# anilkeshwani/speech-integration

Hardware: AMD Instinct MI355X
Metric: train_tokens_per_sec (higher is better)
Workload: dtype bf16; 1 GPU; Llama-3.2-1B +5000 DSUs (V=133258), SFT step fwd+bwd+AdamW, seq_len=2048, batch=8/GPU, grad_accum=1, 16 layers, random-init weights, MLS-shaped synthetic DSU sequences; global_batch=8, seq_len=2048, parallelism=dp1

## Files before the change

### include/ssi_hip.h

```cpp
#ifndef SSI_HIP_H
#define SSI_HIP_H

#include <stdint.h>

#ifdef __cplusplus
extern "C" {
#endif

#define SSI_ABI_VERSION 9

enum { SSI_F32 = 0, SSI_BF16 = 1 };
enum { SSI_OK = 0, SSI_ERR_ARG = 1, SSI_ERR_UNSUPPORTED = 2, SSI_ERR_WORKSPACE = 3, SSI_ERR_HIP = 1000  };
enum { SSI_GEMM_NT = 0, SSI_GEMM_NN = 1, SSI_GEMM_TN = 2 };
enum { SSI_TILES_STATIC = 0, SSI_TILES_DYNAMIC = 1 };
int ssi_set_gemm_tile_order(int mode);

enum { SSI_IMPL_AUTO = 0, SSI_IMPL_GENERIC = 1, SSI_IMPL_MFMA = 2,
       SSI_IMPL_MFMA_WG8 = 3  };

int ssi_abi_version(void);
const char* ssi_last_error(void);
int ssi_set_impl(int impl);

int ssi_embed_fwd(const int64_t* tokens, const void* table, void* out, int64_t n_tok, int64_t dim, int64_t vocab,
                  int dtype, void* stream);
int64_t ssi_embed_bwd_workspace_bytes(int64_t vocab);
int ssi_embed_bwd(const int64_t* tokens, const void* dout, void* dtable, int64_t n_tok, int64_t dim, int64_t vocab,
                  int dtype, void* workspace, int64_t workspace_bytes, void* stream);

int ssi_rmsnorm_fwd(const void* x, const void* scale, void* y, float* rstd, int64_t rows, int64_t dim, float eps,
                    int dtype, void* stream);
int64_t ssi_rmsnorm_bwd_workspace_bytes(int64_t rows, int64_t dim);
int ssi_rmsnorm_bwd(const void* dy, const void* x, const void* scale, const float* rstd, const void* dres, void* dx,
                    void* dscale, int accumulate_dscale, int64_t rows, int64_t dim, int dtype, void* workspace,
                    int64_t workspace_bytes, void* stream);

int ssi_rope_inplace(void* x, int64_t ld, int64_t rows, int64_t seq_len, int n_heads_rot, int head_dim,
                     const float* table, int64_t table_len, const int32_t* positions, int inverse, int dtype,
                     void* stream);

int ssi_gemm_rope(int64_t M, int64_t N, int64_t K, const void* A, int64_t lda, const void* B, int64_t ldb, void* C, int64_t ldc,
                  int64_t seq_len, int n_heads_rot, int head_dim, const float* rope_table, int64_t table_len,
                  const int32_t* positions, int dtype, void* stream);

int ssi_attn_fwd(const void* qkv, int64_t ld, void* out, float* lse, int64_t batch, int64_t seq, int n_heads,
                 int n_kv, int head_dim, int dtype, void* stream);
int ssi_attn_bwd(const void* qkv, int64_t ld, const void* out, const void* dout, const float* lse, void* dqkv,
                 float* delta, int64_t batch, int64_t seq, int n_heads, int n_kv, int head_dim, int dtype,
                 void* stream);

int ssi_attn_varlen_fwd(const void* qkv, int64_t ld, void* out, float* lse, const int32_t* doc_start, const int32_t* doc_end,
                        int64_t batch, int64_t seq, int n_heads, int n_kv, int head_dim, int dtype, void* stream);
int ssi_attn_varlen_bwd(const void* qkv, int64_t ld, const void* out, const void* dout, const float* lse, void* dqkv,
                        float* delta, const int32_t* doc_start, const int32_t* doc_end, int64_t batch, int64_t seq,
                        int n_heads, int n_kv, int head_dim, int dtype, void* stream);

int ssi_doc_ranges(const int64_t* input_pos, int64_t batch, int64_t seq, int64_t max_pos, int32_t* positions, int32_t* doc_start,
                   int32_t* doc_end, int32_t* n_clamped, void* stream);

int ssi_attn_varlen_bwd_rope(const void* qkv, int64_t ld, const void* out, const void* dout, const float* lse, void* dqkv,
                             float* delta, const int32_t* doc_start, const int32_t* doc_end, const float* rope_table,
                             int64_t table_len, const int32_t* positions, int64_t batch, int64_t seq, int n_heads, int n_kv,
                             int head_dim, int dtype, void* stream);

int64_t ssi_attn_bwd_workspace_bytes(int64_t batch, int64_t seq, int n_heads, int n_kv, int head_dim, int dtype);
int ssi_attn_varlen_bwd_ws(const void* qkv, int64_t ld, const void* out, const void* dout, const float* lse, void* dqkv,
                           float* delta, const int32_t* doc_start, const int32_t* doc_end, const float* rope_table,
                           int64_t table_len, const int32_t* positions, int64_t batch, int64_t seq, int n_heads, int n_kv,
                           int head_dim, int dtype, void* workspace, int64_t workspace_bytes, void* stream);

enum { SSI_ATTN_KERNEL_DQ = 0, SSI_ATTN_KERNEL_DKV = 1 };
enum { SSI_ATTN_MODE_AUTO = 0, SSI_ATTN_MODE_OLD = 1, SSI_ATTN_MODE_NEW = 2, SSI_ATTN_MODE_NO_HEAD_SPLIT = 3 };
int ssi_set_attn_impl(int which, int mode);
enum { SSI_ATTN_USED_DQ2 = 1, SSI_ATTN_USED_DKV2 = 2, SSI_ATTN_USED_HEAD_SPLIT = 4, SSI_ATTN_USED_PLAN = 8 };
int ssi_attn_last_dispatch(void);

enum { SSI_ATTN_PLAN_HEADER = 16, SSI_ATTN_PLAN_FORCE = 1, SSI_ATTN_PLAN_SPLIT_ALL = 2  };
int64_t ssi_attn_plan_words(int64_t batch, int64_t seq, int64_t n_docs);
int64_t ssi_attn_plan_workspace_bytes(const int32_t* host_plan_header);
int64_t ssi_attn_plan_build(const int32_t* host_doc_row, const int32_t* host_doc_start, const int32_t* host_doc_end, int64_t n_docs,
                            int64_t batch, int64_t seq, int n_heads, int n_kv, int flags, int32_t* host_plan, int64_t plan_words);
// ... 59 lines not shown
```

### speech-integration_amd/csrc/embed_ce.hip

```cpp
#include "common_hip.h"

template <typename T>
__global__ __launch_bounds__(256) void embed_fwd_kernel(const int64_t* __restrict__ tokens, const T* __restrict__ table,
                                                        T* __restrict__ out, int64_t n_tok, int dim, int64_t vocab) {
    constexpr int N = Vec16<T>::N;
    const int nvec = dim / N;
    for (int64_t t = blockIdx.x; t < n_tok; t += gridDim.x) {
        const int64_t tok = tokens[t];
        const bool ok = tok >= 0 && tok < vocab;
        for (int v = threadIdx.x; v < nvec; v += 256) {
            Vec16<T> a;
            if (ok) a = load16(table + tok * dim + v * N);
            else
#pragma unroll
                for (int i = 0; i < N; ++i) a.set(i, 0.f);
            store16(out + t * dim + v * N, a);
        }
    }
}

extern "C" int ssi_embed_fwd(const int64_t* tokens, const void* table, void* out, int64_t n_tok, int64_t dim,
                             int64_t vocab, int dtype, void* stream) {
    if (n_tok == 0) return SSI_OK;
    SSI_CHECK_ARG(tokens && table && out && n_tok > 0 && dim > 0 && dim % 8 == 0 && vocab > 0);
// ... 85 lines not shown
                for (int k = 0; k < MAXV; ++k) {
                    const bool ok = row_ok && lane + k * 64 < nvec;
#pragma unroll
                    for (int i = 0; i < N; ++i) acc[k][i] += ok ? a[u][k].get(i) : 0.f;
                }
            }
        }
        found += n;
    }
    T* dst = dtable + tok * dim;
#pragma unroll
    for (int k = 0; k < MAXV; ++k) {
        const int v = lane + k * 64;
        if (v < nvec) {
            Vec16<T> a = load16(dst + v * N);
#pragma unroll
            for (int i = 0; i < N; ++i) a.set(i, a.get(i) + acc[k][i]);
            store16(dst + v * N, a);
        }
    }
}

static inline int64_t embed_ws_vocab_slots(int64_t vocab) { return ssi_align_up(vocab, 64); }
extern "C" int64_t ssi_embed_bwd_workspace_bytes(int64_t vocab) { return 2 * embed_ws_vocab_slots(vocab) * (int64_t)sizeof(int); }

template <typename T>
static int launch_embed_bwd(const int64_t* tokens, const T* dout, T* dtable, int64_t n_tok, int dim, int64_t vocab,
                            const int* first, const int* count, hipStream_t st) {
    const int64_t vec_per_lane = ssi_cdiv(dim / Vec16<T>::N, 64);
    const dim3 grid((unsigned)ssi_cdiv(n_tok, 4));
    if (vec_per_lane <= 1) hipLaunchKernelGGL((embed_bwd_kernel<T, 1>), grid, dim3(256), 0, st, tokens, dout, dtable, n_tok, dim, vocab, first, count);
    else if (vec_per_lane <= 2) hipLaunchKernelGGL((embed_bwd_kernel<T, 2>), grid, dim3(256), 0, st, tokens, dout, dtable, n_tok, dim, vocab, first, count);
    else if (vec_per_lane <= 4) hipLaunchKernelGGL((embed_bwd_kernel<T, 4>), grid, dim3(256), 0, st, tokens, dout, dtable, n_tok, dim, vocab, first, count);
    else if (vec_per_lane <= 8) hipLaunchKernelGGL((embed_bwd_kernel<T, 8>), grid, dim3(256), 0, st, tokens, dout, dtable, n_tok, dim, vocab, first, count);
    else { ssi_set_error("embed_bwd: dim %d too large", dim); return SSI_ERR_UNSUPPORTED; }
    return SSI_OK;
}

extern "C" int ssi_embed_bwd(const int64_t* tokens, const void* dout, void* dtable, int64_t n_tok, int64_t dim,
                             int64_t vocab, int dtype, void* workspace, int64_t workspace_bytes, void* stream) {
    if (n_tok == 0) return SSI_OK;
    SSI_CHECK_ARG(tokens && dout && dtable && n_tok > 0 && n_tok < (1LL << 31) && dim > 0 && dim % 8 == 0 && vocab > 0);
    if (!workspace || workspace_bytes < ssi_embed_bwd_workspace_bytes(vocab)) { ssi_set_error("embed_bwd: workspace too small"); return SSI_ERR_WORKSPACE; }
    auto st = (hipStream_t)stream;
    int* first = (int*)workspace;
    int* count = first + embed_ws_vocab_slots(vocab);
    hipError_t e = hipMemsetAsync(first, 0x7f, embed_ws_vocab_slots(vocab) * sizeof(int), st);
    if (e == hipSuccess) e = hipMemsetAsync(count, 0, embed_ws_vocab_slots(vocab) * sizeof(int), st);
    if (e != hipSuccess) { ssi_set_error("embed_bwd: memset failed: %s", hipGetErrorString(e)); return SSI_ERR_HIP + (int)e; }
    hipLaunchKernelGGL(embed_index_kernel, dim3((unsigned)ssi_cdiv(n_tok, 256)), dim3(256), 0, st, tokens, n_tok, vocab, first, count);
    SSI_LAUNCH_CHECK();
    int rc = SSI_OK;
    SSI_DISPATCH_DTYPE(dtype, rc = launch_embed_bwd<T>(tokens, (const T*)dout, (T*)dtable, n_tok, (int)dim, vocab, first, count, st));
    if (rc) return rc;
    SSI_LAUNCH_CHECK();
    return SSI_OK;
}

template <typename T>
__global__ __launch_bounds__(512) void ce_fwd_kernel(T* __restrict__ logits, int64_t ld, const int64_t* __restrict__ labels,
                                                     int64_t vocab, int64_t ignore_index, float* __restrict__ row_loss,
                                                     float* __restrict__ row_lse, int write_grad, const float* __restrict__ row_weight) {
    constexpr int N = Vec16<T>::N;
    __shared__ float red[16];
    const int64_t row = blockIdx.x;
    T* lr = logits + row * ld;
    const int64_t label = labels[row];
    const bool valid = label != ignore_index && label >= 0 && label < vocab;
    const int64_t nvec = ld / N;
    if (!valid) {
        if (threadIdx.x == 0) { row_loss[row] = 0.f; if (row_lse) row_lse[row] = 0.f; }
        if (write_grad) {
            Vec16<T> z;
#pragma unroll
            for (int i = 0; i < N; ++i) z.set(i, 0.f);
            for (int64_t v = threadIdx.x; v < nvec; v += 512) store16(lr + v * N, z);
        }
        return;
    }
    float m = -INFINITY, s = 0.f;
    for (int64_t v = threadIdx.x; v < nvec; v += 512) {
        Vec16<T> a = load16(lr + v * N);
        float lm = -INFINITY;
#pragma unroll
        for (int i = 0; i < N; ++i) if (v * N + i < vocab) lm = fmaxf(lm, a.get(i));
        if (lm > m) { s *= expf(m - lm); m = lm; }
#pragma unroll
        for (int i = 0; i < N; ++i) if (v * N + i < vocab) s += expf(a.get(i) - m);
    }
    const float gm = block_max(m, red);
    s = (m == -INFINITY) ? 0.f : s * expf(m - gm);
    const float gs = block_sum(s, red);
    const float lse = gm + logf(gs);
    const float w = row_weight ? row_weight[row] : 1.f;
    if (threadIdx.x == 0) {
        row_loss[row] = w * (lse - to_f32<T>(lr[label]));
        if (row_lse) row_lse[row] = lse;
    }
    if (!write_grad) return;
    __syncthreads();
    for (int64_t v = threadIdx.x; v < nvec; v += 512) {
        Vec16<T> a = load16(lr + v * N), o;
#pragma unroll
        for (int i = 0; i < N; ++i) {
            const int64_t c = v * N + i;
            float g = 0.f;
// ... 179 lines not shown
```

### speech-integration_amd/ssi/_lib.py

```python

from __future__ import annotations

import ctypes
import os
from ctypes import POINTER, c_char_p, c_double, c_float, c_int, c_int32, c_int64, c_void_p

import torch

_HERE = os.path.dirname(os.path.abspath(__file__))
LIB_PATH = os.environ.get("SSI_HIP_LIB") or os.path.join(os.path.dirname(_HERE), "libssi_hip.so")

SSI_F32, SSI_BF16 = 0, 1
GEMM_NT, GEMM_NN, GEMM_TN = 0, 1, 2
IMPL_AUTO, IMPL_GENERIC, IMPL_MFMA, IMPL_MFMA_WG8 = 0, 1, 2, 3
TILES_STATIC, TILES_DYNAMIC = 0, 1
ABI_VERSION = 9
ATTN_KERNEL_DQ, ATTN_KERNEL_DKV = 0, 1
ATTN_MODE_AUTO, ATTN_MODE_OLD, ATTN_MODE_NEW, ATTN_MODE_NO_HEAD_SPLIT = 0, 1, 2, 3
ATTN_USED_DQ2, ATTN_USED_DKV2, ATTN_USED_HEAD_SPLIT, ATTN_USED_PLAN = 1, 2, 4, 8
ATTN_PLAN_HEADER, ATTN_PLAN_FORCE, ATTN_PLAN_SPLIT_ALL = 16, 1, 2

_P = c_void_p
PROTOTYPES = {
    "ssi_abi_version": (c_int, []),
    "ssi_last_error": (c_char_p, []),
    "ssi_set_impl": (c_int, [c_int]),
    "ssi_set_attn_impl": (c_int, [c_int, c_int]),
    "ssi_attn_last_dispatch": (c_int, []),
    "ssi_embed_fwd": (c_int, [_P, _P, _P, c_int64, c_int64, c_int64, c_int, _P]),
    "ssi_embed_bwd_workspace_bytes": (c_int64, [c_int64]),
    "ssi_embed_bwd": (c_int, [_P, _P, _P, c_int64, c_int64, c_int64, c_int, _P, c_int64, _P]),
    "ssi_rmsnorm_fwd": (c_int, [_P, _P, _P, _P, c_int64, c_int64, c_float, c_int, _P]),
    "ssi_rmsnorm_bwd_workspace_bytes": (c_int64, [c_int64, c_int64]),
    "ssi_rmsnorm_bwd": (c_int, [_P, _P, _P, _P, _P, _P, _P, c_int, c_int64, c_int64, c_int, _P, c_int64, _P]),
    "ssi_rope_inplace": (c_int, [_P, c_int64, c_int64, c_int64, c_int, c_int, _P, c_int64, _P, c_int, c_int, _P]),
    "ssi_gemm_rope": (c_int, [c_int64, c_int64, c_int64, _P, c_int64, _P, c_int64, _P, c_int64, c_int64, c_int, c_int, _P, c_int64, _P,
                              c_int, _P]),
    "ssi_attn_fwd": (c_int, [_P, c_int64, _P, _P, c_int64, c_int64, c_int, c_int, c_int, c_int, _P]),
    "ssi_attn_bwd": (c_int, [_P, c_int64, _P, _P, _P, _P, _P, c_int64, c_int64, c_int, c_int, c_int, c_int, _P]),
    "ssi_set_gemm_tile_order": (c_int, [c_int]),
    "ssi_attn_varlen_fwd": (c_int, [_P, c_int64, _P, _P, _P, _P, c_int64, c_int64, c_int, c_int, c_int, c_int, _P]),
    "ssi_attn_varlen_bwd": (c_int, [_P, c_int64, _P, _P, _P, _P, _P, _P, _P, c_int64, c_int64, c_int, c_int, c_int, c_int, _P]),
    "ssi_attn_varlen_bwd_rope": (c_int, [_P, c_int64, _P, _P, _P, _P, _P, _P, _P, _P, c_int64, _P, c_int64, c_int64, c_int, c_int, c_int,
                                         c_int, _P]),
    "ssi_attn_bwd_workspace_bytes": (c_int64, [c_int64, c_int64, c_int, c_int, c_int, c_int]),
    "ssi_attn_varlen_bwd_ws": (c_int, [_P, c_int64, _P, _P, _P, _P, _P, _P, _P, _P, c_int64, _P, c_int64, c_int64, c_int, c_int, c_int,
                                       c_int, _P, c_int64, _P]),
    "ssi_attn_plan_words": (c_int64, [c_int64, c_int64, c_int64]),
    "ssi_attn_plan_workspace_bytes": (c_int64, [_P]),
    "ssi_attn_plan_build": (c_int64, [_P, _P, _P, c_int64, c_int64, c_int64, c_int, c_int, c_int, _P, c_int64]),
    "ssi_attn_varlen_bwd_plan": (c_int, [_P, c_int64, _P, _P, _P, _P, _P, _P, _P, _P, c_int64, _P, c_int64, c_int64, c_int, c_int, c_int,
                                         c_int, _P, c_int64, _P, _P, _P]),
    "ssi_doc_ranges": (c_int, [_P, c_int64, c_int64, c_int64, _P, _P, _P, _P, _P]),
    "ssi_swiglu_fwd": (c_int, [_P, _P, c_int64, c_int64, c_int, _P]),
    "ssi_swiglu_bwd": (c_int, [_P, _P, _P, c_int64, c_int64, c_int, _P]),
    "ssi_gemm": (c_int, [c_int, c_int64, c_int64, c_int64, _P, c_int64, _P, c_int64, _P, c_int64, _P, c_float, _P,
                         c_int, c_int, _P]),
    "ssi_gemm_splitk_workspace_bytes": (c_int64, [c_int64, c_int64, c_int]),
    "ssi_gemm_splitk": (c_int, [c_int, c_int64, c_int64, c_int64, _P, c_int64, _P, c_int64, _P, c_int64, _P, c_float, _P,
                                c_int, c_int, c_int, _P, c_int64, _P]),
    "ssi_gemm_batched": (c_int, [c_int, c_int, c_int64, c_int64, c_int64, _P, c_int64, c_int64, _P, c_int64, c_int64, _P, c_int64, c_int64,
                                 c_float, _P, c_int, c_int, _P]),
    "ssi_gemm_swiglu_fwd": (c_int, [c_int64, c_int64, c_int64, _P, c_int64, _P, c_int64, _P, c_int64, _P, c_int64, c_int, _P]),
    "ssi_gemm_swiglu_bwd": (c_int, [c_int, c_int64, c_int64, c_int64, _P, c_int64, _P, c_int64, _P, c_int64, _P, c_int64, _P, c_int,
                                    _P]),
    "ssi_transpose": (c_int, [_P, c_int64, _P, c_int64, c_int64, c_int64, c_int, _P]),
    "ssi_ce_fwd": (c_int, [_P, c_int64, _P, c_int64, c_int64, c_int64, _P, _P, c_int, c_int, _P]),
    "ssi_ce_fwd_weighted": (c_int, [_P, c_int64, _P, _P, c_int64, c_int64, c_int64, _P, _P, c_int, c_int, _P]),
    "ssi_ce_reduce": (c_int, [_P, _P, c_int64, c_int64, c_int64, _P, _P]),
    "ssi_lmhead_ce_fwd": (c_int, [_P, c_int64, _P, c_int64, _P, c_int64, c_int64, c_int64, c_int64, c_int64, _P, c_int64, _P, _P, c_int, c_int, _P]),
    "ssi_lmhead_ce_bwd": (c_int, [_P, c_int64, _P, c_int64, _P, c_int64, _P, c_int64, c_int64, c_int64, _P, c_int64, _P, c_int64, c_int, c_int, _P]),
    "ssi_count_tokens": (c_int, [_P, _P, c_int64, _P, c_int, c_int64, c_int64, _P, _P]),
    "ssi_scale_inplace": (c_int, [_P, c_int64, c_float, _P, c_int, _P]),
    "ssi_sumsq_workspace_bytes": (c_int64, [c_int64]),
    "ssi_sumsq": (c_int, [_P, c_int64, c_int, _P, _P, c_int64, _P]),
    "ssi_adamw_step": (c_int, [_P, _P, _P, _P, c_int64, c_double, c_double, c_double, c_double, c_double, c_int64, _P, c_int,
                               c_int, _P]),
}

_lib = None


class HipLibraryError(RuntimeError):
    pass
# ... 55 lines not shown
```

### speech-integration_amd/ssi/model.py

```python

from __future__ import annotations

import os

import logging
import math
from typing import Any, Optional

import torch
from torch import Tensor, nn

from . import _lib, ops
from .constants import CROSS_ENTROPY_IGNORE_IDX, PRECISION_STR_TO_DTYPE
from .llama_configs import ConfigLlama3_2
from .ops import GEMM_NN, GEMM_NT, GEMM_TN

LOGGER = logging.getLogger(__name__)

VOCAB_ALIGN = 256


def _align(n: int, a: int) -> int:
    return (n + a - 1) // a * a

# ... 273 lines not shown
        M, N = c.shape
        K = a.shape[1]
        mfma = self.split_small_grids and self.dtype == torch.bfloat16 and self._mfma_shapes() and M % 256 == 0 and N % 256 == 0
        if mfma and self.split_tail_only and layout in (GEMM_NT, GEMM_NN):
            tm, tn = M // 256, N // 256
            rounds = (tm * tn) // 256
            m_main = (rounds * 256) // tn
            if rounds >= 1 and 0 < m_main < tm and (tm - m_main) * tn <= 192:
                rows = m_main * 256
                ops.gemm(layout, a[:rows], b, c[:rows], residual=None if residual is None else residual[:rows])
                self._gemm(layout, a[rows:], b, c[rows:], None if residual is None else residual[rows:])
                return
        splits = ops.splitk_choice(M, N, K) if mfma else 1
        if splits > 1:
            wsk = self._arena.get("ws.splitk.nt", (splits * M * N,), torch.float32)
            ops.gemm_splitk(layout, a, b, c, splits, wsk, residual=residual)
        else:
            ops.gemm(layout, a, b, c, residual=residual)

    def build_attn_plan(self, input_pos: Tensor, force: bool = False):
        from . import attn_plan
        if input_pos is None or input_pos.is_cuda or input_pos.dim() != 2 or not self._mfma_shapes() or self.head_dim != 64:
            return None
        B, S = input_pos.shape
        if self.num_heads != 4 * self.num_kv_heads or self.padded_seq_len(B, S) != S or S % 128:
            return None
        return attn_plan.plan_from_input_pos(input_pos, self.num_heads, self.num_kv_heads, force=force)

    def _forward_hidden(self, tokens: Tensor, save: bool, input_pos: Optional[Tensor] = None, attn_plan=None) -> Tensor:
        B, S = tokens.shape
        pos = ds = de = None
        self.position_errors = None
        plan = None
        if input_pos is not None and save:
            if attn_plan is None and not input_pos.is_cuda:
                attn_plan = self.build_attn_plan(input_pos)
            if attn_plan is not None and attn_plan.matches(B, S, self.num_heads, self.num_kv_heads) and self._mfma_shapes():
                plan = attn_plan.to_device(tokens.device)
        if input_pos is not None:
            if input_pos.shape != tokens.shape:
                raise ValueError("input_pos must have the shape of tokens")
            if not input_pos.is_cuda and int(input_pos.max()) >= self._rope.shape[0]:
                raise ValueError("input_pos exceeds the RoPE cache")
            self.position_errors = torch.zeros(1, dtype=torch.int32, device=tokens.device)
            pos, ds, de = ops.doc_ranges(input_pos.to(tokens.device), self._rope.shape[0] - 1, self.position_errors)
        T, D, I = B * S, self.embed_dim, self.intermediate_dim
        H, KV, hd, dt, A = self.num_heads, self.num_kv_heads, self.head_dim, self.dtype, self._arena
        if pos is None and S > self._rope.shape[0]:
            raise ValueError(f"sequence length {S} exceeds the RoPE cache ({self._rope.shape[0]})")
        tok = tokens.reshape(-1).contiguous()
        L = self.num_layers
        h = A.get("h0" if save else "h0.x", (T, D), dt)
        ops.embed_fwd(tok, self._view("emb"), h, self.vocab_size)
        for l in range(L):
            sfx = f"{l}" if save else "x"
            xn1 = A.get("xn1.all", (L, T, D), dt)[l] if save else A.get("xn1.x", (T, D), dt)
            rstd1 = A.get(f"rstd1.{sfx}", (T,), torch.float32)
            ops.rmsnorm_fwd(h, self._view(f"L{l}.sa_norm"), xn1, rstd1, self.norm_eps)
            qkv = A.get(f"qkv.{sfx}", (T, self.qkv_dim), dt)
            ops.gemm_rope(xn1, self._view(f"L{l}.wqkv"), qkv, S, H + KV, hd, self._rope, positions=pos)
            att = A.get("att.all", (L, T, H * hd), dt)[l] if save else A.get("att.x", (T, H * hd), dt)
            lse = A.get(f"lse.{sfx}", (B * H * S,), torch.float32)
            ops.attn_fwd(qkv, att, lse, B, S, H, KV, hd, ds, de)
            hmid = A.get(f"hmid.{sfx}", (T, D), dt)
            self._gemm(GEMM_NT, att, self._view(f"L{l}.wo"), hmid, residual=h)
            xn2 = A.get(f"xn2.{sfx}", (T, D), dt)
            rstd2 = A.get(f"rstd2.{sfx}", (T,), torch.float32)
            ops.rmsnorm_fwd(hmid, self._view(f"L{l}.mlp_norm"), xn2, rstd2, self.norm_eps)
            gu = A.get(f"gu.{sfx}", (T, 2 * I), dt)
            act = A.get(f"act.{sfx}", (T, I), dt)
            ops.gemm_swiglu_fwd(xn2, self._view(f"L{l}.w13"), gu, act)
            hn_name = f"h{l + 1}" if save else f"hx{l & 1}"
            hnext = A.get(hn_name, (T, D), dt)
            self._gemm(GEMM_NT, act, self._view(f"L{l}.w2"), hnext, residual=hmid)
            h = hnext
        hn = A.get("hn" if save else "hn.x", (T, D), dt)
        rstdf = A.get("rstdf" if save else "rstdf.x", (T,), torch.float32)
        ops.rmsnorm_fwd(h, self.norm.scale, hn, rstdf, self.norm_eps)
        if save:
            self._fwd_generation += 1
            self._saved = {"tok": tok, "B": B, "S": S, "gen": self._fwd_generation, "pos": pos, "ds": ds, "de": de, "plan": plan}
        return hn

    def _backward_hidden(self, d_hn: Tensor, gen: int) -> None:
        sv = self._saved
        if sv is None or sv["gen"] != gen:
            raise RuntimeError("HipLlamaDecoder: backward called for a forward whose activations were overwritten; "
                               "run backward before the next training forward")
        B, S, tok = sv["B"], sv["S"], sv["tok"]
        pos, ds, de, plan = sv["pos"], sv["ds"], sv["de"], sv.get("plan")
        T, D, I = B * S, self.embed_dim, self.intermediate_dim
        H, KV, hd, dt, A = self.num_heads, self.num_kv_heads, self.head_dim, self.dtype, self._arena
        L = self.num_layers
        G = self._flat_grad
        self._finish_pending_exchange()
        acc = self._window_accumulates()
        gv = lambda name: self._view(name, None, G)
        ws = A.get("ws.rms", (max(ops.rmsnorm_bwd_workspace_bytes(T, D), 16),), torch.uint8)

        def wgrad(dy: Tensor, x: Tensor, name: str) -> None:
            g = gv(name)
            splits = ops.splitk_choice(g.shape[0], g.shape[1], T) if (dt == torch.bfloat16 and T % 64 == 0) else 1
            if splits > 1:
                wsk = A.get("ws.splitk", (splits * g.shape[0] * g.shape[1],), torch.float32)
                ops.gemm_splitk(GEMM_TN, dy, x, g, splits, wsk, accumulate=acc)
            else:
                ops.gemm(GEMM_TN, dy, x, g, accumulate=acc)

        sync = self.grad_sync if (self.grad_sync is not None and self.sync_this_backward) else None
        listener, self.bucket_listener = (self.bucket_listener if self.sync_this_backward else None), None

        def announce(name: str) -> None:
            if sync:
                sync.bucket_ready(*self._bucket_by_name[name])
            if listener is not None:
                listener(*self._bucket_by_name[name])

        Gp = self.wgrad_group
        if sync and Gp != self._bucket_group:
            raise RuntimeError("wgrad_group was changed after construction: the data-parallel buckets were laid out for the old grouping")
        defer = (Gp > 1 and dt == torch.bfloat16 and self._mfma_shapes() and T % 128 == 0 and T >= 256
                 and ops.splitk_choice(D, H * hd, T) > 1 and ops.splitk_choice(self.qkv_dim, D, T) > 1)
        xn1_all, att_all = A.get("xn1.all", (L, T, D), dt), A.get("att.all", (L, T, H * hd), dt)
        if defer:
            dhmid_all, dqkv_all = A.get("dh.b.all", (Gp, T, D), dt), A.get("dqkv.all", (Gp, T, self.qkv_dim), dt)
            lstride = (self._slices["L1.wqkv"][0] - self._slices["L0.wqkv"][0]) if L > 1 else 0

        def flush_attention_wgrads(l_lo: int) -> None:
            n = min(Gp, L - l_lo)
            g_o = torch.as_strided(G, (n, D, H * hd), (lstride, H * hd, 1), self._slices[f"L{l_lo}.wo"][0])
            g_qkv = torch.as_strided(G, (n, self.qkv_dim, D), (lstride, D, 1), self._slices[f"L{l_lo}.wqkv"][0])
            ops.gemm_batched(GEMM_TN, dhmid_all[:n], att_all[l_lo:l_lo + n], g_o, accumulate=acc)
            ops.gemm_batched(GEMM_TN, dqkv_all[:n], xn1_all[l_lo:l_lo + n], g_qkv, accumulate=acc)

        def dgrad(dy: Tensor, name: str, dx: Tensor) -> None:
            self._gemm(GEMM_NN, dy, self._view(name), dx)

        ws_bytes = ops.attn_bwd_workspace_bytes(B, S, H, KV, hd, dt) if T > 0 else 0
        if plan is not None:
            ws_bytes = max(ws_bytes, plan.workspace_bytes)
        attn_ws = A.get("ws.attn", (ws_bytes,), torch.uint8) if ws_bytes else None
        dh = A.get("dh.a", (T, D), dt)
        ops.rmsnorm_bwd(d_hn, A.get(f"h{L}", (T, D), dt), self.norm.scale, A.get("rstdf", (T,), torch.float32), None, dh,
                        gv("norm"), ws, accumulate=acc)
        announce("norm")
        for l in reversed(range(L)):
            xn1, xn2 = xn1_all[l], A.get(f"xn2.{l}", (T, D), dt)
            qkv, att = A.get(f"qkv.{l}", (T, self.qkv_dim), dt), att_all[l]
            hmid, gu, act = A.get(f"hmid.{l}", (T, D), dt), A.get(f"gu.{l}", (T, 2 * I), dt), A.get(f"act.{l}", (T, I), dt)
            h_in = A.get(f"h{l}", (T, D), dt)
            wgrad(dh, act, f"L{l}.w2")
            dgu = A.get("dgu", (T, 2 * I), dt)
            ops.gemm_swiglu_bwd(GEMM_NN, dh, self._view(f"L{l}.w2"), gu, dgu, A.get("dact", (T, I), dt))
            dxn = A.get("dxn", (T, D), dt)
            dgrad(dgu, f"L{l}.w13", dxn)
            wgrad(dgu, xn2, f"L{l}.w13")
            dhmid = dhmid_all[l % Gp] if defer else A.get("dh.b", (T, D), dt)
            ops.rmsnorm_bwd(dxn, hmid, self._view(f"L{l}.mlp_norm"), A.get(f"rstd2.{l}", (T,), torch.float32), dh, dhmid,
                            gv(f"L{l}.mlp_norm"), ws, accumulate=acc)
            datt = A.get("datt", (T, H * hd), dt)
            dgrad(dhmid, f"L{l}.wo", datt)
            if not defer:
                wgrad(dhmid, att, f"L{l}.wo")
            dqkv = dqkv_all[l % Gp] if defer else A.get("dqkv", (T, self.qkv_dim), dt)
            delta = A.get("delta", (B * H * S,), torch.float32)
            ops.attn_bwd(qkv, att, datt, A.get(f"lse.{l}", (B * H * S,), torch.float32), dqkv, delta, B, S, H, KV, hd, ds, de,
                         rope_table=self._rope, positions=pos, workspace=attn_ws, plan=plan)
            dgrad(dqkv, f"L{l}.wqkv", dxn)
            if not defer:
                wgrad(dqkv, xn1, f"L{l}.wqkv")
            ops.rmsnorm_bwd(dxn, h_in, self._view(f"L{l}.sa_norm"), A.get(f"rstd1.{l}", (T,), torch.float32), dhmid, dh,
                            gv(f"L{l}.sa_norm"), ws, accumulate=acc)
            announce(f"L{l}.mlp")
            if defer and l % Gp == 0:
                flush_attention_wgrads(l)
            if l % self._bucket_group == 0:
                announce(f"attn.{l}")
        ws_e = A.get("ws.emb", (max(_lib.load().ssi_embed_bwd_workspace_bytes(self.vocab_size), 16),), torch.uint8)
        if not acc and not self._emb_grad_written:
            gv("emb").zero_()
        ops.embed_bwd(tok, dh, gv("emb"), self.vocab_size, ws_e)
        self._grads_dirty, self._grads_stale, self._emb_grad_written = True, False, False
        announce("emb")
        self._saved = None
        self.attach_grads()

    def _head_logits(self, hn: Tensor, arena_name: Optional[str] = None) -> Tensor:
        T = hn.shape[0]
        if arena_name is None:
            logits = torch.empty((T, self.vocab_pad), dtype=self.dtype, device=self.device)
        else:
            logits = self._arena.get(arena_name, (T, self.vocab_pad), self.dtype)
        ops.gemm(GEMM_NT, hn, self._view("emb"), logits)
        return logits

    def _head_backward(self, dlogits: Tensor, hn: Tensor, alpha_dev: Optional[Tensor]) -> Tensor:
        T, D = hn.shape
        self._finish_pending_exchange()
        acc = self._window_accumulates()
        d_hn = self._arena.get("d_hn", (T, D), self.dtype)
        ops.gemm(GEMM_NN, dlogits, self._view("emb"), d_hn, alpha_dev=alpha_dev)
        g_emb = self._view("emb", None, self._flat_grad)
        rows_main = self._head_wgrad_main_rows(T)
        if rows_main:
            Vp = self.vocab_pad
            ops.gemm(GEMM_TN, dlogits[:, :rows_main], hn, g_emb[:rows_main], alpha_dev=alpha_dev, accumulate=acc)
            tail, splits = Vp - rows_main, self._head_wgrad_tail_splits
            wsk = self._arena.get("ws.splitk.head", (splits * tail * D,), torch.float32)
            ops.gemm_splitk(GEMM_TN, dlogits[:, rows_main:], hn, g_emb[rows_main:], splits, wsk, alpha_dev=alpha_dev, accumulate=acc)
        else:
            ops.gemm(GEMM_TN, dlogits, hn, g_emb, alpha_dev=alpha_dev, accumulate=acc)
        self._emb_grad_written = True
        return d_hn

    _head_wgrad_tail_splits = 3

    def _head_wgrad_main_rows(self, T: int, n_cu: int = 256) -> int:
        if os.environ.get("SSI_HEAD_WGRAD_TAIL", "1") == "0" or self.dtype != torch.bfloat16 or not self._mfma_shapes() or T % 128 or T < 64 * 6 * self._head_wgrad_tail_splits:
            return 0
        tm, tn = self.vocab_pad // 256, self.embed_dim // 256
        full_rounds = (tm * tn) // n_cu
        if full_rounds == 0 or (full_rounds * n_cu) % tn:
            return 0
        tail_tiles = tm * tn - full_rounds * n_cu
        if tail_tiles == 0 or 2 * tail_tiles >= n_cu or tail_tiles * self._head_wgrad_tail_splits > n_cu:
            return 0
        return full_rounds * n_cu // tn * 256

    def _check_inputs(self, tokens: Tensor, mask, encoder_input, encoder_mask, input_pos) -> Tensor:
        if encoder_input is not None or encoder_mask is not None:
            raise NotImplementedError("no encoder inputs: the reference's model is decoder-only (ssi/model.py:34)")
        if mask is not None and input_pos is None:
            raise NotImplementedError("a dense attention mask is never materialised: packed batches pass input_pos, from which "
                                      "the block-causal mask follows (ssi/data/packed.py)")
# ... 174 lines not shown
```

### speech-integration_amd/ssi/ops.py

```python

from __future__ import annotations

import torch
from typing import Optional
from torch import Tensor

from . import _lib
from ._lib import GEMM_NN, GEMM_NT, GEMM_TN, check, dtype_code, ptr, stream_ptr

__all__ = ["lmhead_ce_fwd", "lmhead_ce_bwd", "doc_ranges", "embed_fwd", "embed_bwd", "rmsnorm_fwd", "rmsnorm_bwd", "rope_", "attn_fwd", "attn_bwd", "attn_bwd_workspace_bytes", "swiglu_fwd",
           "swiglu_bwd", "gemm", "gemm_splitk", "splitk_choice", "gemm_swiglu_fwd", "gemm_swiglu_bwd", "transpose", "ce_fwd", "ce_reduce", "count_tokens", "scale_", "sumsq", "adamw_step", "set_impl", "set_attn_impl", "attn_last_dispatch",
           "GEMM_NT", "GEMM_NN", "GEMM_TN"]


def set_impl(impl: int) -> int:
    return _lib.load().ssi_set_impl(impl)


def set_attn_impl(which: int, mode: int) -> int:
    return _lib.load().ssi_set_attn_impl(which, mode)


def attn_last_dispatch() -> int:
    return _lib.load().ssi_attn_last_dispatch()


def _byte_ws(nbytes: int, like: Tensor) -> Tensor:
    return torch.empty(max(int(nbytes), 16), dtype=torch.uint8, device=like.device)


def embed_fwd(tokens: Tensor, table: Tensor, out: Tensor, vocab: int) -> None:
    n, dim = tokens.numel(), table.shape[1]
    assert tokens.dtype == torch.int64 and tokens.is_contiguous() and out.is_contiguous() and table.stride(1) == 1
    assert table.stride(0) == dim and out.shape[-1] == dim and out.numel() == n * dim and out.dtype == table.dtype
    check(_lib.load().ssi_embed_fwd(ptr(tokens), ptr(table), ptr(out), n, dim, vocab, dtype_code(table.dtype),
                                    stream_ptr()), "ssi_embed_fwd")


def embed_bwd(tokens: Tensor, dout: Tensor, dtable: Tensor, vocab: int, workspace: Tensor | None = None) -> None:
    lib = _lib.load()
    n, dim = tokens.numel(), dtable.shape[1]
    assert tokens.dtype == torch.int64 and tokens.is_contiguous() and dout.is_contiguous() and dtable.stride(0) == dim
    need = lib.ssi_embed_bwd_workspace_bytes(vocab)
    if workspace is None or workspace.numel() * workspace.element_size() < need:
        workspace = _byte_ws(need, dout)
    check(lib.ssi_embed_bwd(ptr(tokens), ptr(dout), ptr(dtable), n, dim, vocab, dtype_code(dtable.dtype), ptr(workspace),
                            workspace.numel() * workspace.element_size(), stream_ptr()), "ssi_embed_bwd")


def rmsnorm_fwd(x: Tensor, scale: Tensor, y: Tensor, rstd: Tensor | None, eps: float) -> None:
    dim = x.shape[-1]
    rows = x.numel() // dim
    assert x.is_contiguous() and y.is_contiguous() and scale.is_contiguous() and scale.numel() == dim
    assert rstd is None or (rstd.dtype == torch.float32 and rstd.numel() >= rows)
    check(_lib.load().ssi_rmsnorm_fwd(ptr(x), ptr(scale), ptr(y), ptr(rstd), rows, dim, eps, dtype_code(x.dtype),
                                      stream_ptr()), "ssi_rmsnorm_fwd")


def rmsnorm_bwd_workspace_bytes(rows: int, dim: int) -> int:
    return _lib.load().ssi_rmsnorm_bwd_workspace_bytes(rows, dim)


def rmsnorm_bwd(dy: Tensor, x: Tensor, scale: Tensor, rstd: Tensor, dres: Tensor | None, dx: Tensor, dscale: Tensor,
                workspace: Tensor | None = None, accumulate: bool = True) -> None:
    lib = _lib.load()
    dim = x.shape[-1]
    rows = x.numel() // dim
    assert dy.is_contiguous() and x.is_contiguous() and dx.is_contiguous() and dscale.is_contiguous()
    assert dres is None or dres.is_contiguous()
    need = lib.ssi_rmsnorm_bwd_workspace_bytes(rows, dim)
    if workspace is None or workspace.numel() * workspace.element_size() < need:
        workspace = _byte_ws(need, dy)
    check(lib.ssi_rmsnorm_bwd(ptr(dy), ptr(x), ptr(scale), ptr(rstd), ptr(dres), ptr(dx), ptr(dscale), int(accumulate), rows, dim,
                              dtype_code(x.dtype), ptr(workspace), workspace.numel() * workspace.element_size(),
                              stream_ptr()), "ssi_rmsnorm_bwd")


def rope_(x: Tensor, seq_len: int, n_heads_rot: int, head_dim: int, table: Tensor, inverse: bool = False,
          positions: Tensor | None = None) -> None:
    assert x.dim() == 2 and x.stride(1) == 1 and table.dtype == torch.float32 and table.is_contiguous()
    assert positions is None or (positions.dtype == torch.int32 and positions.numel() == x.shape[0])
    check(_lib.load().ssi_rope_inplace(ptr(x), x.stride(0), x.shape[0], seq_len, n_heads_rot, head_dim, ptr(table),
                                       table.shape[0], ptr(positions), int(inverse), dtype_code(x.dtype), stream_ptr()),
          "ssi_rope_inplace")


def gemm_rope(a: Tensor, b: Tensor, c: Tensor, seq_len: int, n_heads_rot: int, head_dim: int, table: Tensor,
              positions: Tensor | None = None) -> None:
    assert a.dim() == 2 and b.dim() == 2 and c.dim() == 2 and a.stride(1) == 1 and b.stride(1) == 1 and c.stride(1) == 1
    M, K = a.shape
    N = b.shape[0]
    assert b.shape[1] == K and c.shape == (M, N) and a.dtype == b.dtype == c.dtype
    assert table.dtype == torch.float32 and table.is_contiguous() and table.shape[1] * 2 == head_dim
    assert positions is None or (positions.dtype == torch.int32 and positions.numel() == M)
    check(_lib.load().ssi_gemm_rope(M, N, K, ptr(a), a.stride(0), ptr(b), b.stride(0), ptr(c), c.stride(0), seq_len, n_heads_rot, head_dim,
                                    ptr(table), table.shape[0], ptr(positions), dtype_code(a.dtype), stream_ptr()), "ssi_gemm_rope")


def _doc_ptrs(doc_start: Optional[Tensor], doc_end: Optional[Tensor], rows: int):
    if doc_start is None and doc_end is None:
# ... 254 lines not shown
```

Baseline: 150,200 tokens/s.

## Build token-grouping plan in forward and use it for embedding backward

Adds a multi-kernel plan builder that groups token positions by vocabulary id (count, allocate segments, fill, sort) during the forward pass. A new planned embedding-backward kernel then sums gradient rows per distinct token, with dedicated blocks for heavy tokens. This replaces the per-step memsets of vocab-sized workspace and the index kernel in backward. The cost is extra forward-time launches and a self-cleaning scratch buffer that depends on the sort kernel resetting counts.

```diff
diff --git a/include/ssi_hip.h b/include/ssi_hip.h
--- a/include/ssi_hip.h
+++ b/include/ssi_hip.h
@@ -7,7 +7,7 @@
 extern "C" {
 #endif
 
-#define SSI_ABI_VERSION 9
+#define SSI_ABI_VERSION 10
 
 enum { SSI_F32 = 0, SSI_BF16 = 1 };
 enum { SSI_OK = 0, SSI_ERR_ARG = 1, SSI_ERR_UNSUPPORTED = 2, SSI_ERR_WORKSPACE = 3, SSI_ERR_HIP = 1000  };
@@ -27,6 +27,10 @@
 int64_t ssi_embed_bwd_workspace_bytes(int64_t vocab);
 int ssi_embed_bwd(const int64_t* tokens, const void* dout, void* dtable, int64_t n_tok, int64_t dim, int64_t vocab,
                   int dtype, void* workspace, int64_t workspace_bytes, void* stream);
+int64_t ssi_embed_plan_bytes(int64_t n_tok, int64_t vocab);
+int ssi_embed_plan_build(const int64_t* tokens, int64_t n_tok, int64_t vocab, void* plan, int64_t plan_bytes, void* stream);
+int ssi_embed_bwd_planned(const void* plan, const void* dout, void* dtable, int64_t n_tok, int64_t dim, int64_t vocab, int dtype,
+                          void* stream);
 
 int ssi_rmsnorm_fwd(const void* x, const void* scale, void* y, float* rstd, int64_t rows, int64_t dim, float eps,
                     int dtype, void* stream);
diff --git a/speech-integration_amd/csrc/embed_ce.hip b/speech-integration_amd/csrc/embed_ce.hip
--- a/speech-integration_amd/csrc/embed_ce.hip
+++ b/speech-integration_amd/csrc/embed_ce.hip
@@ -161,6 +161,283 @@
     SSI_LAUNCH_CHECK();
     int rc = SSI_OK;
     SSI_DISPATCH_DTYPE(dtype, rc = launch_embed_bwd<T>(tokens, (const T*)dout, (T*)dtable, n_tok, (int)dim, vocab, first, count, st));
+    if (rc) return rc;
+    SSI_LAUNCH_CHECK();
+    return SSI_OK;
+}
+
+constexpr int EP_HDR = 16, EP_HEAVY = 32;
+enum { EP_NDIST = 0, EP_NHEAVY = 1, EP_NTASK = 2, EP_C_NDIST = 8, EP_C_CURSOR = 9, EP_C_NHEAVY = 10, EP_C_NTASK = 11 };
+
+struct EmbedPlan {
+    int *hdr, *cnt, *rank, *ids, *seg_off, *seg_cnt, *raw, *pos, *heavy, *task;
+    int heavy_cap, task_cap;
+    int64_t words;
+};
+
+static EmbedPlan embed_plan_layout(const void* base, int64_t n_tok, int64_t vocab) {
+    EmbedPlan p;
+    int* w = (int*)base;
+    int64_t o = 0;
+    auto take = [&](int64_t n) { int* r = w + o; o += ssi_align_up(n, 4); return r; };
+    p.hdr = take(EP_HDR);
+    p.cnt = take(vocab);
+    p.rank = take(n_tok);
+    p.ids = take(n_tok);
+    p.seg_off = take(n_tok);
+    p.seg_cnt = take(n_tok);
+    p.raw = take(n_tok);
+    p.pos = take(n_tok);
+    p.heavy_cap = (int)(n_tok / EP_HEAVY + 1);
+    p.heavy = take(p.heavy_cap);
+    p.task_cap = (int)(n_tok / 64 + 1);
+    p.task = take(2 * (int64_t)p.task_cap);
+    p.words = o;
+    return p;
+}
+
+__device__ __forceinline__ int wave_claim(int* counter, int n) {
+    const int lane = threadIdx.x & 63;
+    int incl = n;
+#pragma unroll
+    for (int o = 1; o < 64; o <<= 1) {
+        const int up = __shfl_up(incl, o, 64);
+        if (lane >= o) incl += up;
+    }
+    const int total = __shfl(incl, 63, 64);
+    int base = 0;
+    if (lane == 0 && total > 0) base = atomicAdd(counter, total);
+    return __shfl(base, 0, 64) + incl - n;
+}
+
+__global__ __launch_bounds__(256) void embed_plan_count_kernel(const int64_t* __restrict__ tokens, int n_tok, int64_t vocab, EmbedPlan p) {
+    const int t = blockIdx.x * 256 + threadIdx.x;
+    const int64_t tok = tokens[t < n_tok ? t : n_tok - 1];
+    const bool ok = t < n_tok && tok >= 0 && tok < vocab;
+    int r = -1;
+    if (ok) {
+        r = atomicAdd(&p.cnt[tok], 1);
+        p.rank[t] = r;
+    }
+    const int d = wave_claim(&p.hdr[EP_C_NDIST], r == 0 ? 1 : 0);
+    if (r == 0 && (unsigned)d < (unsigned)n_tok) p.ids[d] = (int)tok;
+}
+
+__global__ __launch_bounds__(256) void embed_plan_alloc_kernel(int n_tok, int64_t vocab, EmbedPlan p) {
+    const int d = blockIdx.x * 256 + threadIdx.x;
+    int nd = p.hdr[EP_C_NDIST];
+    nd = (unsigned)nd < (unsigned)n_tok ? nd : n_tok;
+    if (d == 0) p.hdr[EP_NDIST] = nd;
+    if ((d & ~63) >= nd) return;
+    const int tok = d < nd ? p.ids[d] : -1;
+    const bool ok = tok >= 0 && tok < vocab;
+    int c = ok ? p.cnt[tok] : 0;
+    if (c < 0 || c > n_tok) c = 0;
+    const int off = wave_claim(&p.hdr[EP_C_CURSOR], c);
+    if (d >= nd) return;
+    p.seg_off[d] = off;
+    p.seg_cnt[d] = c;
+    if (!ok) return;
+    p.cnt[tok] = off;
+    if (c >= EP_HEAVY) {
+        const int h = atomicAdd(&p.hdr[EP_C_NHEAVY], 1);
+        if ((unsigned)h < (unsigned)p.heavy_cap) p.heavy[h] = d;
+    }
+    if (c > 64) {
+        const int nt = (c - 1) / 64;
+        const int tb = atomicAdd(&p.hdr[EP_C_NTASK], nt);
+        for (int k = 0; k < nt; ++k)
+            if ((unsigned)(tb + k) < (unsigned)p.task_cap) { p.task[2 * (tb + k)] = d; p.task[2 * (tb + k) + 1] = k + 1; }
+    }
+}
+
+__global__ __launch_bounds__(256) void embed_plan_fill_kernel(const int64_t* __restrict__ tokens, int n_tok, int64_t vocab, EmbedPlan p) {
+    const int t = blockIdx.x * 256 + threadIdx.x;
+    if (t == 0) {
+        const int nh = p.hdr[EP_C_NHEAVY], nt = p.hdr[EP_C_NTASK];
+        p.hdr[EP_NHEAVY] = (unsigned)nh < (unsigned)p.heavy_cap ? nh : p.heavy_cap;
+        p.hdr[EP_NTASK] = (unsigned)nt < (unsigned)p.task_cap ? nt : p.task_cap;
+        p.hdr[EP_C_NDIST] = p.hdr[EP_C_CURSOR] = p.hdr[EP_C_NHEAVY] = p.hdr[EP_C_NTASK] = 0;
+    }
+    if (t >= n_tok) return;
+    const int64_t tok = tokens[t];
+    if (tok < 0 || tok >= vocab) return;
+    const int idx = p.cnt[tok] + p.rank[t];
+    if ((unsigned)idx < (unsigned)n_tok) p.raw[idx] = t;
+}
+
+__global__ __launch_bounds__(256) void embed_plan_sort_kernel(int n_tok, int64_t vocab, EmbedPlan p) {
+    const int lane = threadIdx.x & 63;
+    const int w = blockIdx.x * 4 + (threadIdx.x >> 6);
+    int d, k = 0;
+    if (w < n_tok) {
+        d = w;
+        if (d >= p.hdr[EP_NDIST]) return;
+    } else {
+        const int tk = w - n_tok;
+        if (tk >= p.hdr[EP_NTASK]) return;
+        d = p.task[2 * tk];
+        k = p.task[2 * tk + 1];
+        if ((unsigned)d >= (unsigned)n_tok) return;
+    }
+    d = __builtin_amdgcn_readfirstlane(d);
+    k = __builtin_amdgcn_readfirstlane(k);
+    const int off = __builtin_amdgcn_readfirstlane(p.seg_off[d]);
+    const int c = __builtin_amdgcn_readfirstlane(p.seg_cnt[d]);
+    const int tok = __builtin_amdgcn_readfirstlane(p.ids[d]);
+    if (tok < 0 || tok >= vocab) return;
+    if (k == 0 && lane == 0) p.cnt[tok] = 0;
+    if (off < 0 || c <= 0 || c > n_tok - off || k * 64 >= c) return;
+    const int* raw = p.raw + off;
+    const int i = k * 64 + lane;
+    const int e = raw[i < c ? i : c - 1];
+    int rk = 0;
+    for (int jb = 0; jb < c; jb += 64) {
+        const int x = raw[jb + lane < c ? jb + lane : c - 1];
+        const int n = c - jb < 64 ? c - jb : 64;
+        for (int j = 0; j < n; ++j) rk += __builtin_amdgcn_readlane(x, j) < e ? 1 : 0;
+    }
+    if (i < c) p.pos[off + rk] = e;
+}
+
+extern "C" int64_t ssi_embed_plan_bytes(int64_t n_tok, int64_t vocab) {
+    if (n_tok < 0 || vocab <= 0) return -1;
+    return embed_plan_layout(nullptr, n_tok, vocab).words * (int64_t)sizeof(int);
+}
+
+extern "C" int ssi_embed_plan_build(const int64_t* tokens, int64_t n_tok, int64_t vocab, void* plan, int64_t plan_bytes, void* stream) {
+    if (n_tok == 0) return SSI_OK;
+    SSI_CHECK_ARG(tokens && n_tok > 0 && n_tok < (1LL << 30) && vocab > 0 && vocab < (1LL << 31) && ((uintptr_t)plan & 3) == 0);
+    if (!plan || plan_bytes < ssi_embed_plan_bytes(n_tok, vocab)) { ssi_set_error("embed_plan_build: plan buffer too small"); return SSI_ERR_WORKSPACE; }
+    auto st = (hipStream_t)stream;
+    const EmbedPlan p = embed_plan_layout(plan, n_tok, vocab);
+    const int n = (int)n_tok;
+    const dim3 per_tok((unsigned)ssi_cdiv(n_tok, 256));
+    hipLaunchKernelGGL(embed_plan_count_kernel, per_tok, dim3(256), 0, st, tokens, n, vocab, p);
+    hipLaunchKernelGGL(embed_plan_alloc_kernel, per_tok, dim3(256), 0, st, n, vocab, p);
+    hipLaunchKernelGGL(embed_plan_fill_kernel, per_tok, dim3(256), 0, st, tokens, n, vocab, p);
+    hipLaunchKernelGGL(embed_plan_sort_kernel, dim3((unsigned)ssi_cdiv(n_tok + p.task_cap, 4)), dim3(256), 0, st, n, vocab, p);
+    SSI_LAUNCH_CHECK();
+    return SSI_OK;
+}
+
+template <typename T, int MAXV, int ROWS>
+__device__ __forceinline__ void embed_add_rows(const T* __restrict__ dout, int dim, int n_tok, int pl, int h0, int c, const int (&vcl)[MAXV],
+                                               const bool (&vok)[MAXV], float (&acc)[MAXV][Vec16<T>::N]) {
+    constexpr int N = Vec16<T>::N;
+    Vec16<T> a[ROWS][MAXV];
+#pragma unroll
+    for (int u = 0; u < ROWS; ++u) {
+        const int h = h0 + u < c ? h0 + u : c - 1;
+        const int t = __builtin_amdgcn_readlane(pl, h & 63);
+        const T* src = dout + (int64_t)((unsigned)t < (unsigned)n_tok ? t : 0) * dim;
+#pragma unroll
+        for (int k = 0; k < MAXV; ++k) a[u][k] = load16(src + vcl[k] * N);
+    }
+    __builtin_amdgcn_sched_barrier(0);
+#pragma unroll
+    for (int u = 0; u < ROWS; ++u) {
+        const bool row_ok = h0 + u < c;
+#pragma unroll
+        for (int k = 0; k < MAXV; ++k) {
+            const bool ok = row_ok && vok[k];
+#pragma unroll
+            for (int i = 0; i < N; ++i) acc[k][i] += ok ? a[u][k].get(i) : 0.f;
+        }
+    }
+}
+
+template <typename T, int MAXV>
+__global__ __launch_bounds__(256) void embed_bwd_planned_kernel(EmbedPlan p, const T* __restrict__ dout, T* __restrict__ dtable, int n_tok,
+                                                                int dim, int64_t vocab) {
+    constexpr int N = Vec16<T>::N;
+    const int lane = threadIdx.x & 63, wave = threadIdx.x >> 6;
+    const int nvec = dim / N;
+    if ((int)blockIdx.x < p.heavy_cap) {
+        if ((int)blockIdx.x >= p.hdr[EP_NHEAVY]) return;
+        const int d = __builtin_amdgcn_readfirstlane(p.heavy[blockIdx.x]);
+        if ((unsigned)d >= (unsigned)n_tok) return;
+        const int off = __builtin_amdgcn_readfirstlane(p.seg_off[d]), c = __builtin_amdgcn_readfirstlane(p.seg_cnt[d]);
+        const int64_t tok = __builtin_amdgcn_readfirstlane(p.ids[d]);
+        if (off < 0 || c <= 0 || c > n_tok - off || tok < 0 || tok >= vocab) return;
+        constexpr int DEEP = 32;
+        for (int s = wave; s * 64 < nvec; s += 4) {
+            const int v = s * 64 + lane;
+            const int vcl[1] = {v < nvec ? v : nvec - 1};
+            const bool vok[1] = {v < nvec};
+            T* dst = dtable + tok * dim + vcl[0] * N;
+            Vec16<T> b = load16(dst);
+            float acc[1][N];
+#pragma unroll
+            for (int i = 0; i < N; ++i) acc[0][i] = 0.f;
+            for (int jb = 0; jb < c; jb += 64) {
+                const int pl = p.pos[off + (jb + lane < c ? jb + lane : c - 1)];
+                embed_add_rows<T, 1, DEEP>(dout, dim, n_tok, pl, 0, c - jb, vcl, vok, acc);
+                if (jb + DEEP < c) embed_add_rows<T, 1, DEEP>(dout, dim, n_tok, pl, DEEP, c - jb, vcl, vok, acc);
+            }
+            if (vok[0]) {
+#pragma unroll
+                for (int i = 0; i < N; ++i) b.set(i, b.get(i) + acc[0][i]);
+                store16(dst, b);
+            }
+        }
+        return;
+    }
+    const int d = ((int)blockIdx.x - p.heavy_cap) * 4 + wave;
+    if (d >= p.hdr[EP_NDIST]) return;
+    const int c = __builtin_amdgcn_readfirstlane(p.seg_cnt[d]);
+    if (c >= EP_HEAVY) return;
+    const int off = __builtin_amdgcn_readfirstlane(p.seg_off[d]);
+    const int64_t tok = __builtin_amdgcn_readfirstlane(p.ids[d]);
+    if (off < 0 || c <= 0 || c > n_tok - off || tok < 0 || tok >= vocab) return;
+    const int pl = p.pos[off + (lane < c ? lane : c - 1)];
+    int vcl[MAXV];
+    bool vok[MAXV];
+    float acc[MAXV][N];
+    Vec16<T> b[MAXV];
+    T* dst = dtable + tok * dim;
+#pragma unroll
+    for (int k = 0; k < MAXV; ++k) {
+        const int v = lane + k * 64;
+        vok[k] = v < nvec;
+        vcl[k] = vok[k] ? v : nvec - 1;
+        b[k] = load16(dst + vcl[k] * N);
+#pragma unroll
+        for (int i = 0; i < N; ++i) acc[k][i] = 0.f;
+    }
+    if (c == 1) embed_add_rows<T, MAXV, 1>(dout, dim, n_tok, pl, 0, c, vcl, vok, acc);
+    else if (c <= 4) embed_add_rows<T, MAXV, 4>(dout, dim, n_tok, pl, 0, c, vcl, vok, acc);
+    else
+        for (int h0 = 0; h0 < c; h0 += 8) embed_add_rows<T, MAXV, 8>(dout, dim, n_tok, pl, h0, c, vcl, vok, acc);
+#pragma unroll
+    for (int k = 0; k < MAXV; ++k)
+        if (vok[k]) {
+#pragma unroll
+            for (int i = 0; i < N; ++i) b[k].set(i, b[k].get(i) + acc[k][i]);
+            store16(dst + vcl[k] * N, b[k]);
+        }
+}
+
+template <typename T>
+static int launch_embed_bwd_planned(const EmbedPlan& p, const T* dout, T* dtable, int64_t n_tok, int dim, int64_t vocab, hipStream_t st) {
+    const int64_t vec_per_lane = ssi_cdiv(dim / Vec16<T>::N, 64);
+    const dim3 grid((unsigned)(p.heavy_cap + ssi_cdiv(n_tok, 4)));
+    if (vec_per_lane <= 1) hipLaunchKernelGGL((embed_bwd_planned_kernel<T, 1>), grid, dim3(256), 0, st, p, dout, dtable, (int)n_tok, dim, vocab);
+    else if (vec_per_lane <= 2) hipLaunchKernelGGL((embed_bwd_planned_kernel<T, 2>), grid, dim3(256), 0, st, p, dout, dtable, (int)n_tok, dim, vocab);
+    else if (vec_per_lane <= 4) hipLaunchKernelGGL((embed_bwd_planned_kernel<T, 4>), grid, dim3(256), 0, st, p, dout, dtable, (int)n_tok, dim, vocab);
+    else if (vec_per_lane <= 8) hipLaunchKernelGGL((embed_bwd_planned_kernel<T, 8>), grid, dim3(256), 0, st, p, dout, dtable, (int)n_tok, dim, vocab);
+    else { ssi_set_error("embed_bwd_planned: dim %d too large", dim); return SSI_ERR_UNSUPPORTED; }
+    return SSI_OK;
+}
+
+extern "C" int ssi_embed_bwd_planned(const void* plan, const void* dout, void* dtable, int64_t n_tok, int64_t dim, int64_t vocab, int dtype,
+                                     void* stream) {
+    if (n_tok == 0) return SSI_OK;
+    SSI_CHECK_ARG(plan && dout && dtable && n_tok > 0 && n_tok < (1LL << 30) && dim > 0 && dim % 8 == 0 && vocab > 0 && vocab < (1LL << 31) &&
+                  ((uintptr_t)plan & 3) == 0);
+    const EmbedPlan p = embed_plan_layout(plan, n_tok, vocab);
+    int rc = SSI_OK;
+    SSI_DISPATCH_DTYPE(dtype, rc = launch_embed_bwd_planned<T>(p, (const T*)dout, (T*)dtable, n_tok, (int)dim, vocab, (hipStream_t)stream));
     if (rc) return rc;
     SSI_LAUNCH_CHECK();
     return SSI_OK;
diff --git a/speech-integration_amd/ssi/_lib.py b/speech-integration_amd/ssi/_lib.py
--- a/speech-integration_amd/ssi/_lib.py
+++ b/speech-integration_amd/ssi/_lib.py
@@ -14,7 +14,7 @@
 GEMM_NT, GEMM_NN, GEMM_TN = 0, 1, 2
 IMPL_AUTO, IMPL_GENERIC, IMPL_MFMA, IMPL_MFMA_WG8 = 0, 1, 2, 3
 TILES_STATIC, TILES_DYNAMIC = 0, 1
-ABI_VERSION = 9
+ABI_VERSION = 10
 ATTN_KERNEL_DQ, ATTN_KERNEL_DKV = 0, 1
 ATTN_MODE_AUTO, ATTN_MODE_OLD, ATTN_MODE_NEW, ATTN_MODE_NO_HEAD_SPLIT = 0, 1, 2, 3
 ATTN_USED_DQ2, ATTN_USED_DKV2, ATTN_USED_HEAD_SPLIT, ATTN_USED_PLAN = 1, 2, 4, 8
@@ -30,6 +30,9 @@
     "ssi_embed_fwd": (c_int, [_P, _P, _P, c_int64, c_int64, c_int64, c_int, _P]),
     "ssi_embed_bwd_workspace_bytes": (c_int64, [c_int64]),
     "ssi_embed_bwd": (c_int, [_P, _P, _P, c_int64, c_int64, c_int64, c_int, _P, c_int64, _P]),
+    "ssi_embed_plan_bytes": (c_int64, [c_int64, c_int64]),
+    "ssi_embed_plan_build": (c_int, [_P, c_int64, c_int64, _P, c_int64, _P]),
+    "ssi_embed_bwd_planned": (c_int, [_P, _P, _P, c_int64, c_int64, c_int64, c_int, _P]),
     "ssi_rmsnorm_fwd": (c_int, [_P, _P, _P, _P, c_int64, c_int64, c_float, c_int, _P]),
     "ssi_rmsnorm_bwd_workspace_bytes": (c_int64, [c_int64, c_int64]),
     "ssi_rmsnorm_bwd": (c_int, [_P, _P, _P, _P, _P, _P, _P, c_int, c_int64, c_int64, c_int, _P, c_int64, _P]),
diff --git a/speech-integration_amd/ssi/model.py b/speech-integration_amd/ssi/model.py
--- a/speech-integration_amd/ssi/model.py
+++ b/speech-integration_amd/ssi/model.py
@@ -349,6 +349,13 @@
         L = self.num_layers
         h = A.get("h0" if save else "h0.x", (T, D), dt)
         ops.embed_fwd(tok, self._view("emb"), h, self.vocab_size)
+        eplan = None
+        if save and T > 0:
+            held = A.buf.get("emb.plan")
+            eplan = A.get("emb.plan", (ops.embed_plan_bytes(T, self.vocab_size),), torch.uint8)
+            if A.buf["emb.plan"] is not held:
+                A.buf["emb.plan"].zero_()
+            ops.embed_plan_build(tok, self.vocab_size, eplan)
         for l in range(L):
             sfx = f"{l}" if save else "x"
             xn1 = A.get("xn1.all", (L, T, D), dt)[l] if save else A.get("xn1.x", (T, D), dt)
@@ -376,7 +383,7 @@
         ops.rmsnorm_fwd(h, self.norm.scale, hn, rstdf, self.norm_eps)
         if save:
             self._fwd_generation += 1
-            self._saved = {"tok": tok, "B": B, "S": S, "gen": self._fwd_generation, "pos": pos, "ds": ds, "de": de, "plan": plan}
+            self._saved = {"tok": tok, "B": B, "S": S, "gen": self._fwd_generation, "pos": pos, "ds": ds, "de": de, "plan": plan, "eplan": eplan}
         return hn
 
     def _backward_hidden(self, d_hn: Tensor, gen: int) -> None:
@@ -473,10 +480,13 @@
                 flush_attention_wgrads(l)
             if l % self._bucket_group == 0:
                 announce(f"attn.{l}")
-        ws_e = A.get("ws.emb", (max(_lib.load().ssi_embed_bwd_workspace_bytes(self.vocab_size), 16),), torch.uint8)
         if not acc and not self._emb_grad_written:
             gv("emb").zero_()
-        ops.embed_bwd(tok, dh, gv("emb"), self.vocab_size, ws_e)
+        if sv.get("eplan") is not None:
+            ops.embed_bwd_planned(sv["eplan"], T, dh, gv("emb"), self.vocab_size)
+        else:
+            ws_e = A.get("ws.emb", (max(_lib.load().ssi_embed_bwd_workspace_bytes(self.vocab_size), 16),), torch.uint8)
+            ops.embed_bwd(tok, dh, gv("emb"), self.vocab_size, ws_e)
         self._grads_dirty, self._grads_stale, self._emb_grad_written = True, False, False
         announce("emb")
         self._saved = None
diff --git a/speech-integration_amd/ssi/ops.py b/speech-integration_amd/ssi/ops.py
--- a/speech-integration_amd/ssi/ops.py
+++ b/speech-integration_amd/ssi/ops.py
@@ -8,7 +8,7 @@
 from . import _lib
 from ._lib import GEMM_NN, GEMM_NT, GEMM_TN, check, dtype_code, ptr, stream_ptr
 
-__all__ = ["lmhead_ce_fwd", "lmhead_ce_bwd", "doc_ranges", "embed_fwd", "embed_bwd", "rmsnorm_fwd", "rmsnorm_bwd", "rope_", "attn_fwd", "attn_bwd", "attn_bwd_workspace_bytes", "swiglu_fwd",
+__all__ = ["lmhead_ce_fwd", "lmhead_ce_bwd", "doc_ranges", "embed_fwd", "embed_bwd", "embed_plan_bytes", "embed_plan_build", "embed_bwd_planned", "embed_plan_read", "rmsnorm_fwd", "rmsnorm_bwd", "rope_", "attn_fwd", "attn_bwd", "attn_bwd_workspace_bytes", "swiglu_fwd",
            "swiglu_bwd", "gemm", "gemm_splitk", "splitk_choice", "gemm_swiglu_fwd", "gemm_swiglu_bwd", "transpose", "ce_fwd", "ce_reduce", "count_tokens", "scale_", "sumsq", "adamw_step", "set_impl", "set_attn_impl", "attn_last_dispatch",
            "GEMM_NT", "GEMM_NN", "GEMM_TN"]
 
@@ -46,6 +46,36 @@
         workspace = _byte_ws(need, dout)
     check(lib.ssi_embed_bwd(ptr(tokens), ptr(dout), ptr(dtable), n, dim, vocab, dtype_code(dtable.dtype), ptr(workspace),
                             workspace.numel() * workspace.element_size(), stream_ptr()), "ssi_embed_bwd")
+
+
+def embed_plan_bytes(n_tok: int, vocab: int) -> int:
+    return int(_lib.load().ssi_embed_plan_bytes(n_tok, vocab))
+
+
+def embed_plan_build(tokens: Tensor, vocab: int, plan: Tensor) -> None:
+    assert tokens.dtype == torch.int64 and tokens.is_contiguous() and plan.is_contiguous()
+    check(_lib.load().ssi_embed_plan_build(ptr(tokens), tokens.numel(), vocab, ptr(plan), plan.numel() * plan.element_size(),
+                                           stream_ptr()), "ssi_embed_plan_build")
+
+
+def embed_bwd_planned(plan: Tensor, n_tok: int, dout: Tensor, dtable: Tensor, vocab: int) -> None:
+    dim = dtable.shape[1]
+    assert dout.is_contiguous() and dtable.stride(0) == dim and dout.numel() == n_tok * dim and dout.dtype == dtable.dtype
+    assert plan.numel() * plan.element_size() >= embed_plan_bytes(n_tok, vocab)
+    check(_lib.load().ssi_embed_bwd_planned(ptr(plan), ptr(dout), ptr(dtable), n_tok, dim, vocab, dtype_code(dtable.dtype),
+                                            stream_ptr()), "ssi_embed_bwd_planned")
+
+
+def embed_plan_read(plan: Tensor, n_tok: int, vocab: int) -> dict:
+    w = plan.view(torch.uint8)[:embed_plan_bytes(n_tok, vocab)].view(torch.int32).cpu()
+    pad, o, arr = (lambda n: (n + 3) // 4 * 4), 0, {}
+    for name, n in (("hdr", 16), ("cnt", vocab), ("rank", n_tok), ("ids", n_tok), ("seg_off", n_tok), ("seg_cnt", n_tok), ("raw", n_tok),
+                    ("pos", n_tok), ("heavy", n_tok // 32 + 1)):
+        arr[name], o = w[o:o + n], o + pad(n)
+    nd, nh = int(arr["hdr"][0]), int(arr["hdr"][1])
+    ids, off, cnt = arr["ids"][:nd].tolist(), arr["seg_off"][:nd].tolist(), arr["seg_cnt"][:nd].tolist()
+    return {"lists": {i: arr["pos"][s:s + c].tolist() for i, s, c in zip(ids, off, cnt)},
+            "heavy": sorted(ids[d] for d in arr["heavy"][:nh].tolist()), "scratch_clean": not bool(arr["cnt"].any()) and not bool(arr["hdr"][8:].any())}
 
 
 def rmsnorm_fwd(x: Tensor, scale: Tensor, y: Tensor, rstd: Tensor | None, eps: float) -> None:
```

Measured after the change: 150,600 tokens/s (median of 3 runs). No clear change (+0.2%).
